# Lillthorin/YoloLite-Official-Repo

Hardware: AMD Instinct MI355X
Metric: images/sec (higher is better)
Workload: dtype f32

## Files before the change

### yololite-official-repo_amd/_lib.py

```python
from __future__ import annotations

import ctypes as C
import os
import sys
import warnings


def _default_hw_queues():
    if "GPU_MAX_HW_QUEUES" in os.environ or os.environ.get("YOLOLITE_NO_ENV_DEFAULTS"):
        return
    os.environ["GPU_MAX_HW_QUEUES"] = "8"
    t = sys.modules.get("torch")
    try:
        late = t is not None and t.cuda.is_initialized()
    except Exception:
        late = False
    if late:
        warnings.warn("yololite_amd: the HIP runtime was initialised before this package was imported, so "
                      "GPU_MAX_HW_QUEUES=8 cannot be applied; export it in the environment (multi-stream overlap "
                      "of the executor degrades by ~25 % next to RCCL streams otherwise)", RuntimeWarning)


_default_hw_queues()

_HERE = os.path.dirname(os.path.abspath(__file__))
LIB_PATH = os.environ.get("YOLOLITE_HIP_LIB") or os.path.join(_HERE, "libyololite_hip.so")

YL_ABI_VERSION = 5
YL_MAX_LEVELS = 8
YL_OK = 0
ACT = {"none": 0, "relu": 1, "relu6": 2, "silu": 3, "gelu": 4, "relu_lab": 5}
OP_STEM, OP_CONV, OP_DW, OP_STEMBLOCK, OP_SE = 0, 1, 2, 3, 4
OP_POOL, OP_COPY, OP_LN, OP_GRN, OP_NHWC4 = 5, 6, 7, 8, 9
POST_MAIN, POST_FALLBACK, POST_EVAL = 0, 1, 2
CENTER = {"v8": 0, "simple": 1}
WH = {"softplus": 0, "v8": 1, "exp": 2}
NMS_TORCHVISION, NMS_GREEDY = 0, 1

DEV_DW_TILE_OFF, DEV_PWS_OFF, DEV_S2C_OFF, DEV_DWC_ALL, DEV_DWT_OFF = 1, 2, 4, 8, 16
DEV_DWT_NOSPLIT = 1 << 10
DEV_WINO_V1 = 1 << 11
DEV_DWL_OFF = 1 << 14
DEV_DWL_ALL = 1 << 15
DEV_DPW_OFF = 1 << 16
DEV_K3W_OFF = 1 << 17
DEV_POISON = 1 << 18
DEV_CHAIN_OFF = 1 << 19
DEV_WINO_SHAPE_SHIFT = 12

_fp = C.POINTER(C.c_float)
_ip = C.POINTER(C.c_int32)


class yl_layer(C.Structure):
    _fields_ = [(n, C.c_int32) for n in (
        "op", "in_slot", "out_slot", "res_slot", "up_slot", "head_level", "cin", "cout",
        "k", "stride", "pad_t", "pad_l", "act", "in_shift", "dw_k", "dw_stride", "dw_pad_t", "dw_pad_l", "dw_act")] + [
        ("w", _fp), ("b", _fp), ("dw_w", _fp), ("dw_b", _fp),
        ("c2", C.c_int32), ("act2", C.c_int32), ("c3", C.c_int32), ("act3", C.c_int32),
        ("w2", _fp), ("b2", _fp), ("w3", _fp), ("b3", _fp), ("scale_slot", C.c_int32), ("reserved0", C.c_int32),
        ("lab_scale", C.c_float), ("lab_bias", C.c_float), ("eps", C.c_float), ("out_ch_off", C.c_int32)]


class yl_model_desc(C.Structure):
    _fields_ = [("abi_version", C.c_int32), ("img_size", C.c_int32), ("in_channels", C.c_int32),
                ("num_classes", C.c_int32), ("num_masks", C.c_int32), ("proto_slot", C.c_int32),
                ("num_levels", C.c_int32),
                ("level_size", C.c_int32 * YL_MAX_LEVELS), ("level_anchors", C.c_int32 * YL_MAX_LEVELS),
                ("num_slots", C.c_int32), ("slot_h", _ip), ("slot_w", _ip), ("slot_c", _ip),
                ("num_layers", C.c_int32), ("layers", C.POINTER(yl_layer))]


class yl_post_cfg(C.Structure):
    _fields_ = [("mode", C.c_int32), ("conf_thr", C.c_float), ("iou_thr", C.c_float),
                ("per_class_cap", C.c_int32), ("topk", C.c_int32), ("max_out", C.c_int32),
                ("center_mode", C.c_int32), ("wh_mode", C.c_int32), ("backmap_dev", C.c_void_p),
                ("fallback_nms", C.c_int32)]


YL_LOSS_MAX_TOPK = 64
# ... 98 lines not shown
```

### yololite-official-repo_amd/csrc/yl_api.hip

```cpp
#include "yl_internal.h"

#include <dlfcn.h>
#include <limits.h>
#include <math.h>
#include <stdio.h>
#include <stddef.h>
#include <string.h>

#include <algorithm>
#include <memory>
#include <chrono>
#include <string>
#include <vector>

#define YL_DW_LDS_MAX (32 * 1024)

namespace {

struct DevLayer {
  yl_layer d;
  float* wp = nullptr;
  float* bias = nullptr;
  float* dw_w = nullptr;
  float* dw_b = nullptr;
// ... 46 lines not shown
  float* level_buf[YL_MAX_LEVELS] = {nullptr};
  float4* ws_boxes = nullptr;
  float* ws_scores = nullptr;
  int* ws_cls = nullptr;
  int* ws_clsws = nullptr;
  int* ws_kept_list = nullptr;
  int* ws_done = nullptr;
  unsigned long long* ws_gkeys = nullptr;
  int gP = 0;
  float* ws_tmp_dets = nullptr;
  int* ws_tmp_idx = nullptr;
  int post_cap_batch = 0;
  unsigned long long* ws_loss_keys = nullptr;
  float* ws_loss_neg = nullptr;
  float* ws_loss_pi = nullptr;
  int* ws_loss_pos = nullptr;
  int loss_cap_batch = 0;
  int* ws_nms_clsws = nullptr;
  unsigned long long* ws_nms_gkeys = nullptr;
  int nms_gP = 0;
  int opt_graph = 0, opt_tile_m = 0, opt_streams = 2;
  int opt_nms_groups = 0;
  int opt_hybrid = 0;
  int small_lo = 0, small_hi = 0;
  int tiny_lo = 0, tiny_hi = 0;
  int opt_batch_levels = 1;
  int opt_winograd = 1;
  int wino_max_hw = 0;
  int opt_fuse_decode = 1;
  int opt_fuse_head = 1;
  int opt_split_k = 0;
  int opt_dev = 0;
  int chain_launches = 0;
  int opt_bf16 = 0;
  hipStream_t work[4] = {nullptr, nullptr, nullptr, nullptr};
  hipEvent_t ev_fork = nullptr, ev_join[4] = {nullptr, nullptr, nullptr, nullptr};
  int opt_lanes = 0;
  std::vector<unsigned char> lane;
  std::vector<int> readers;
  hipStream_t side[4] = {nullptr, nullptr, nullptr, nullptr};
  hipEvent_t ev_la[4] = {nullptr, nullptr, nullptr, nullptr}, ev_lb[4] = {nullptr, nullptr, nullptr, nullptr};
  struct GraphEntry {
    std::vector<hipGraphExec_t> execs;
    int n = 0;
    std::vector<unsigned char> key;
    unsigned long long stamp = 0;
  };
  std::vector<GraphEntry> graphs;
  unsigned long long graph_clock = 0;
  std::shared_ptr<int> weights_owner;
  std::string err;
};

namespace {

bool g_inited[64] = {false};

yl_status fail(yl_ctx* c, yl_status s, const std::string& msg) {
  if (c) c->err = msg;
  return s;
}

#define HIPCHK(ctx, expr)                                                                        \
  do {                                                                                           \
    hipError_t _e = (expr);                                                                      \
    if (_e != hipSuccess) {                                                                      \
// ... 496 lines not shown
};
#define YL_MODE_LAUNCHERS(S, SD)                                                                             \
  {yl_launch_conv##S, yl_launch_conv_multi##S, yl_launch_stem##SD, yl_launch_dw##SD, yl_launch_stemblock##S, \
   yl_launch_stemdw##S, yl_conv_init##S, yl_convc_init##S, yl_stemblock_init##S}
const ModeLaunchers kLaunch[4] = {YL_MODE_LAUNCHERS(, ), YL_MODE_LAUNCHERS(_bf16, ), YL_MODE_LAUNCHERS(_f16, ),
                                  YL_MODE_LAUNCHERS(_f16s, _f16s)};

yl_status launch_failed(yl_ctx* c, const LaunchStep& s, hipError_t e) {
  static const char* const what[] = {"", "batched ", "head ", "expand-only ", "fused ", "chained ", "split head "};
  char b[256];
  snprintf(b, sizeof(b), "layers %zu..%zu %slaunch failed: %s", s.first, s.first + s.layers - 1, what[s.form], hipGetErrorString(e));
  return fail(c, YL_ERR_HIP, b);
}

struct LayerRun {
  yl_ctx* c;
  const float* x; int b0, B; float* const* level_out;
  hipStream_t st; hipEvent_t* evs; int chunk; const yl_post_cfg* fuse; size_t lend;
  bool lanes = false;
  hipStream_t sd = nullptr;
  std::vector<unsigned char> prod;
  bool side_used = false;
  int pooled_slot = -1, pooled_P = 0;

  void decode_targets(size_t i, YlConvP& p) const {
    const int l = c->layers[i].d.head_level, S = c->level_S[l];
    const size_t o = (size_t)b0 * c->N;
    p.dec_boxes = c->ws_boxes + o; p.dec_scores = c->ws_scores + o; p.dec_cls = c->ws_cls + o;
    p.dec_N = c->N; p.dec_off = c->level_off[l] + c->layers[i].head_anchor * S * S; p.dec_C = c->C;
    p.dec_mode = fuse->mode; p.dec_center = fuse->center_mode; p.dec_wh = fuse->wh_mode;
    p.dec_raw = c->NM > 0 ? 1 : 0;
    p.dec_stride = (float)((double)c->img_size / (double)S);
    p.dec_hi = (float)(c->img_size - 1);
  }
  void params(size_t i, YlConvP& p) const {
    layer_params(c, c->layers[i], b0, B, x, level_out, p);
    if (fuse && c->layers[i].d.head_level >= 0) decode_targets(i, p);
  }
};

yl_status run_layer(LayerRun& r, size_t i) {
  yl_ctx* c = r.c;
  const DevLayer& L = c->layers[i];
  const yl_layer& d = L.d;
  const int b0 = r.b0, B = r.B;
  const ModeLaunchers& ml = kLaunch[c->opt_bf16];
  YlConvP p;
  r.params(i, p);
  const int ln = (r.lanes && c->lane[i]) ? 1 : 0;
  hipStream_t ls = ln ? r.sd : r.st;
  if (r.lanes) {
    bool cross = false;
    const int ins[4] = {d.in_slot, d.res_slot, d.up_slot, d.scale_slot};
    for (int k = 0; k < 4; ++k)
      if (ins[k] >= 0 && d.op != YL_OP_STEM && d.op != YL_OP_STEMBLOCK && d.op != YL_OP_NHWC4 && r.prod[ins[k]] != ln) cross = true;
    if (ln == 1 && !r.side_used) cross = true;
    if (cross) {
      hipEvent_t ev = ln ? c->ev_la[r.chunk] : c->ev_lb[r.chunk];
      HIPCHK(c, hipEventRecord(ev, ln ? r.st : r.sd));
      HIPCHK(c, hipStreamWaitEvent(ls, ev, 0));
    }
    if (ln) r.side_used = true;
    if (d.head_level < 0 && d.out_slot >= 0) r.prod[d.out_slot] = (unsigned char)ln;
  }
  hipError_t e;
  switch (d.op) {
// ... 47 lines not shown
      break;
    case YL_OP_STEMBLOCK: e = d.dw_k == 3 ? ml.stemdw(p, ls) : ml.stemblock(p, ls); break;
    default: e = ml.dw(p, ls); break;
  }
  if (e == hipSuccess && YL_ACT_POSTPASS(d.act) && c->opt_bf16 == 3) return fail(c, YL_ERR_UNSUPPORTED, "store_f16: GELU / ReLU + affine passes are fp32-storage only");
  if (e == hipSuccess && YL_ACT_POSTPASS(d.act)) {
    YlOpP q;
    memset(&q, 0, sizeof(q));
    q.x = p.out; q.out = p.out;
    q.B = B; q.OH = L.out_h; q.OW = L.out_w; q.C = d.cout;
    q.act = d.act; q.lab_s = d.lab_scale; q.lab_b = d.lab_bias;
    if (d.res_slot >= 0) q.res = slot_addr(c, d.res_slot, b0);
    e = yl_launch_op(YL_OP_ACTPASS, q, ls);
  }
  if (e != hipSuccess) return launch_failed(c, {F_LAYER, i, 1, 1}, e);
  if (r.evs) HIPCHK(c, hipEventRecord(r.evs[i + 1], r.st));
  return YL_OK;
}

yl_status emit(LayerRun& r, const LaunchStep& s, bool* refused) {
  yl_ctx* c = r.c;
  const size_t i = s.first, n = (size_t)s.width;
  hipError_t e = hipSuccess;
  YlConvP ps[4];
  switch (s.form) {
    case F_LAYER: return run_layer(r, i);
    case F_HEAD_RUN:
      for (size_t q = 0; q < n; ++q) {
        const DevLayer& O = c->layers[i + n + q];
        r.params(i + q, ps[q]);
        ps[q].w3p = O.wp; ps[q].b3 = O.bias; ps[q].C3 = O.d.cout;
        r.decode_targets(i + n + q, ps[q]);
      }
      e = yl_launch_conv_dpp(ps, (int)n, r.st);
      break;
    case F_DPQ_EXPAND:
      r.params(i, ps[0]);
      ps[0].w3p = nullptr;
      e = yl_launch_conv_dpq(ps[0], r.st);
      break;
    case F_DPQ_PAIR: case F_DWX_CHAIN: {
      YlConvP& pt = ps[0]; YlConvP& po = ps[1];
      r.params(i, pt);
      r.params(i + 1, po);
      pt.w3p = po.wp; pt.b3 = po.bias; pt.C3 = po.N; pt.act3 = po.act;
      if (s.form == F_DPQ_PAIR) { pt.res = po.res; pt.out = po.out; }
      e = s.form == F_DPQ_PAIR ? yl_launch_conv_dpq(pt, r.st) : yl_launch_conv_dwx(pt, po.out, r.st);
      if (s.form == F_DWX_CHAIN && e == hipSuccess) ++c->chain_launches;
      break;
    }
    case F_SPLIT_HEAD: case F_BATCHED:
      for (size_t q = 0; q < n; ++q) {
        r.params(i + q, ps[q]);
        if (s.form == F_BATCHED) continue;
        const DevLayer& L = c->layers[i + q];
        YlConvP& a = ps[q];
        const int nd = 5 + c->C;
        a.wp = L.wp_det; a.bias = L.b_det; a.N = nd; a.NTtot = cdiv(nd, 16); a.dec_raw = 0;
        a.w3p = L.wp_mc; a.b3 = L.b_mc; a.C3 = c->NM;
        a.out += nd; a.ldo = c->E;
      }
      e = kLaunch[c->opt_bf16].conv_multi(ps, (int)n, c->opt_tile_m, r.st);
      break;
  }
  const unsigned fused = form_bit(F_HEAD_RUN) | form_bit(F_DPQ_EXPAND) | form_bit(F_DPQ_PAIR) | form_bit(F_DWX_CHAIN);
  *refused = e == hipErrorNotSupported && (fused & form_bit(s.form));
  if (e != hipSuccess && !*refused) return launch_failed(c, s, e);
// ... 353 lines not shown
  return walk_plan(c, j, st, n, segs, nseg, [&](int g, int i, int, int, hipStream_t ws) -> yl_status {
    HIPCHK(c, hipGraphLaunch(ge->execs[first[g] + i], ws));
    return YL_OK;
  });
}

}

extern "C" {

int32_t yl_abi_version(void) { return YL_ABI_VERSION; }

const char* yl_strerror(yl_status s) {
  switch (s) {
    case YL_OK: return "ok";
    case YL_ERR_INVALID: return "invalid argument";
    case YL_ERR_HIP: return "HIP runtime error";
    case YL_ERR_NOMEM: return "out of memory";
    case YL_ERR_STATE: return "invalid state for this call";
    case YL_ERR_UNSUPPORTED: return "unsupported configuration";
    case YL_ERR_CAPACITY: return "output buffer too small";
    default: return "unknown yl_status";
  }
}

const char* yl_last_error(const yl_ctx* ctx) { return ctx ? ctx->err.c_str() : "null context"; }

void yl_destroy(yl_ctx* c) {
  if (!c) return;
  hipSetDevice(c->device);
  free_act(c);
  free_post_ws(c);
  hipFree(c->ws_nms_clsws);
  hipFree(c->ws_loss_keys); hipFree(c->ws_loss_neg); hipFree(c->ws_loss_pi); hipFree(c->ws_loss_pos);
  for (int i = 0; i < 4; ++i) {
    if (c->work[i]) hipStreamDestroy(c->work[i]);
    if (c->ev_join[i]) hipEventDestroy(c->ev_join[i]);
    if (c->side[i]) hipStreamDestroy(c->side[i]);
    if (c->ev_la[i]) hipEventDestroy(c->ev_la[i]);
    if (c->ev_lb[i]) hipEventDestroy(c->ev_lb[i]);
  }
  if (c->ev_fork) hipEventDestroy(c->ev_fork);
  for (int i = 0; i < 3; ++i) if (c->ev_t[i]) hipEventDestroy(c->ev_t[i]);
  hipFree(c->ws_nms_gkeys);
  if (c->weights_owner.use_count() <= 1) {
    hipFree(c->zeros);
    for (auto& L : c->layers) {
      hipFree(L.wp); hipFree(L.bias); hipFree(L.dw_w); hipFree(L.dw_b);
      hipFree(L.w2p); hipFree(L.b2); hipFree(L.w3p); hipFree(L.b3); hipFree(L.wino);
      hipFree(L.wp_det); hipFree(L.b_det); hipFree(L.wp_mc); hipFree(L.b_mc);
    }
  }
  delete c;
}

yl_status yl_clone(const yl_ctx* src, yl_ctx** out) {
  if (!src || !out) return YL_ERR_INVALID;
  *out = nullptr;
  if (hipSetDevice(src->device) != hipSuccess) return YL_ERR_HIP;
  yl_ctx* c = new (std::nothrow) yl_ctx();
  if (!c) return YL_ERR_NOMEM;
  *out = c;
  c->device = src->device;
  c->img_size = src->img_size; c->in_ch = src->in_ch; c->C = src->C; c->L = src->L; c->N = src->N; c->E = src->E;
  c->NM = src->NM; c->proto_slot = src->proto_slot;
  memcpy(c->level_S, src->level_S, sizeof(c->level_S));
// ... 356 lines not shown
  return YL_OK;
}

yl_status yl_set_option(yl_ctx* c, const char* name, int32_t value) {
  if (!c || !name) return YL_ERR_INVALID;
  if (!strcmp(name, "graph")) { c->opt_graph = value ? 1 : 0; drop_graph(c); return YL_OK; }
  if (!strcmp(name, "mfma_bf16")) { if (c->opt_bf16 == 3) free_act(c); c->opt_bf16 = value ? 1 : (c->opt_bf16 == 1 ? 0 : c->opt_bf16); drop_graph(c); return YL_OK; }
  if (!strcmp(name, "mfma_f16")) { if (c->opt_bf16 == 3) free_act(c); c->opt_bf16 = value ? 2 : (c->opt_bf16 == 2 ? 0 : c->opt_bf16); drop_graph(c); return YL_OK; }
  if (!strcmp(name, "store_f16")) {
    const int nv = value ? 3 : (c->opt_bf16 == 3 ? 0 : c->opt_bf16);
    if ((nv == 3) != (c->opt_bf16 == 3)) free_act(c);
    c->opt_bf16 = nv; drop_graph(c); return YL_OK;
  }
  if (!strcmp(name, "nms_groups")) { c->opt_nms_groups = value < 0 ? 0 : (value > YL_NMS_GROUPS ? YL_NMS_GROUPS : value); drop_graph(c); return YL_OK; }
  if (!strcmp(name, "time_split")) {
    c->opt_time_split = value ? 1 : 0;
    for (int i = 0; i < 3 && value; ++i)
      if (!c->ev_t[i]) HIPCHK(c, hipEventCreate(&c->ev_t[i]));
    c->timing_valid = false;
    return YL_OK;
  }
  if (!strcmp(name, "pre_norm")) { c->opt_pre_norm = value ? 1 : 0; return YL_OK; }
  if (!strcmp(name, "reuse_slots")) { c->opt_reuse = value ? 1 : 0; drop_graph(c); return YL_OK; }
  if (!strcmp(name, "hybrid")) { c->opt_hybrid = value < 0 ? 0 : (value > 2 ? 2 : value); drop_graph(c); return YL_OK; }
  if (!strcmp(name, "batch_levels")) { c->opt_batch_levels = value ? 1 : 0; drop_graph(c); return YL_OK; }
  if (!strcmp(name, "fuse_decode")) { c->opt_fuse_decode = value ? 1 : 0; drop_graph(c); return YL_OK; }
  if (!strcmp(name, "fuse_head")) { c->opt_fuse_head = value ? 1 : 0; drop_graph(c); return YL_OK; }
  if (!strcmp(name, "winograd")) { c->opt_winograd = value < 0 ? 0 : (value > 2 ? 2 : value); drop_graph(c); return YL_OK; }
  if (!strcmp(name, "lanes")) { c->opt_lanes = value ? 1 : 0; drop_graph(c); return YL_OK; }
  if (!strcmp(name, "tile_m")) { c->opt_tile_m = value; drop_graph(c); return YL_OK; }
  if (!strcmp(name, "streams")) { c->opt_streams = value < 1 ? 1 : (value > 4 ? 4 : value); drop_graph(c); return YL_OK; }
  if (!strcmp(name, "split_k")) { c->opt_split_k = value ? 1 : 0; drop_graph(c); return YL_OK; }
  if (!strcmp(name, "dev_select")) { c->opt_dev = value & (int)YL_DEV_MASK; drop_graph(c); return YL_OK; }
  return fail(c, YL_ERR_INVALID, std::string("unknown option ") + name);
}

yl_status yl_get_option(const yl_ctx* c, const char* name, int32_t* value) {
  if (!c || !name || !value) return YL_ERR_INVALID;
  const struct { const char* n; int v; } tab[] = {
      {"graph", c->opt_graph}, {"mfma_bf16", c->opt_bf16 == 1}, {"mfma_f16", c->opt_bf16 == 2}, {"store_f16", c->opt_bf16 == 3}, {"nms_groups", c->opt_nms_groups}, {"time_split", c->opt_time_split},
      {"pre_norm", c->opt_pre_norm}, {"reuse_slots", c->opt_reuse}, {"hybrid", c->opt_hybrid}, {"batch_levels", c->opt_batch_levels},
      {"fuse_decode", c->opt_fuse_decode}, {"fuse_head", c->opt_fuse_head}, {"winograd", c->opt_winograd}, {"lanes", c->opt_lanes},
      {"tile_m", c->opt_tile_m}, {"streams", c->opt_streams}, {"dev_select", c->opt_dev}, {"split_k", c->opt_split_k},
      {"chain_launches", c->chain_launches}};
  for (const auto& t : tab)
    if (!strcmp(name, t.n)) { *value = t.v; return YL_OK; }
  return YL_ERR_INVALID;
}

int32_t yl_query_fused_block(int32_t c_in, int32_t c_mid, int32_t c_out, int32_t dw_k, int32_t dw_stride, int32_t out_h,
                             int32_t out_w) {
  if (c_in < 1 || c_mid < 1 || c_out < 1 || out_h < 1 || out_w < 1) return 0;
  if (yl_ir_supported(c_in, c_mid, c_out, dw_k, dw_stride, out_h, out_w)) return 1;
  if (dw_stride == 1 && !(out_h & 3) && !(out_w & 3) && yl_uib_supported(c_in, c_mid, c_out, dw_k)) return 2;
  return 0;
}

int32_t yl_query_dw_prologue(int32_t c_in, int32_t c_out, int32_t dw_k, int32_t dw_stride, int32_t out_h, int32_t out_w) {
  if (c_in < 1 || c_out < 1 || dw_k < 1 || dw_stride < 1 || out_h < 1 || out_w < 1) return 0;
  if (yl_dws_supported(c_in, c_out, dw_k, dw_stride, out_h, out_w)) return 2;
  if ((size_t)(dw_k * dw_k + 1) * c_in * sizeof(float) <= YL_DW_LDS_MAX) return 1;
  return 0;
}

static yl_status forward_impl(yl_ctx* c, const float* x, int B, float* const* level_out, hipStream_t st,
                              float* layer_ms, const yl_post_cfg* cfg, float* dets, int* counts, int* keep_idx = nullptr) {
  if (!c) return YL_ERR_INVALID;
  if (c->layers.empty()) return fail(c, YL_ERR_STATE, "context was created without layers");
  if (!x || B < 1) return fail(c, YL_ERR_INVALID, "bad input");
  HIPCHK(c, hipSetDevice(c->device));
  yl_status s = ensure_act(c, B, layer_ms ? 1 : chunks_for(c, B));
  if (s != YL_OK) return s;
  if (cfg && (s = ensure_post(c, B)) != YL_OK) return s;
  if ((s = poison_act(c, st)) != YL_OK) return s;
  Job j;
  j.x = x; j.B = B; j.cfg = cfg; j.dets = dets; j.counts = counts; j.keep_idx = keep_idx;
  for (int l = 0; l < c->L; ++l) j.outs[l] = (level_out && level_out[l]) ? level_out[l] : c->level_buf[l];
  if (layer_ms) {
    std::vector<hipEvent_t> ev(c->layers.size() + 1);
// ... 289 lines not shown
```

### yololite-official-repo_amd/csrc/yl_dpp.hip

```cpp
#include <stdlib.h>
#include "yl_internal.h"
#include "yl_dev.h"
#include "yl_epi.h"

constexpr int DPP_NW = 8;
constexpr int DPW_NW = 8;
constexpr int DPP_WPE = 2;

struct YlDppLds {
  static constexpr int WSL = 192;
  static constexpr __host__ __device__ int nbuf(int KB) { return (KB % 3 == 0) ? 3 : 2; }
  size_t w3, dw, b1, b3, win, bytes;
  constexpr __host__ __device__ YlDppLds(int KB, int NT1, int NT3, bool bias3, int ring_f4)
      : w3((size_t)KB * NT1 * 256), dw(w3 + (size_t)NT1 * NT3 * 256), b1(dw + 10 * KB * 16), b3(b1 + NT1 * 16),
        win(b3 + (bias3 ? NT3 * 16 : 0)), bytes((win + (size_t)ring_f4 * 4) * 4) {}
  static constexpr __host__ __device__ YlDppLds dpp(int KB, int NT1, int NT3) { return YlDppLds(KB, NT1, NT3, true, 0); }
  static constexpr __host__ __device__ YlDppLds dpw(int KB, int NT1, int NT3) { return YlDppLds(KB, NT1, NT3, true, DPW_NW * nbuf(KB) * WSL); }
  static constexpr __host__ __device__ YlDppLds dpq(int KB, int NC1, int NT3) { return YlDppLds(KB, NC1 * 6, NT3, false, 0); }
};

template <int KB , int NT1 , int NT3 >
__global__ __launch_bounds__(DPP_NW * 64, DPP_WPE) void yl_conv_dpp_kernel(YlConvMulti mp) {
  int yl_k = 0;
  if (mp.n > 1 && (int)blockIdx.x >= mp.p[1].blk0) yl_k = 1;
// ... 92 lines not shown
      }
      yl_mma_step<NT1, 1>(wq, xq, acc1);
      xq[0] = xn;
      asm volatile("" ::: "memory");
    };
#pragma unroll
    for (int kb = 0; kb < KB; kb += 2) {
      block(xb, kb);
      if (kb + 1 < KB) block(xa, kb + 1);
    }
    const int next = tile + DPP_NW;
    if (next < r1) { setup(next); fetch(xa, 0); }
    f32x4 acc3[1][NT3];
#pragma unroll
    for (int nt = 0; nt < NT3; ++nt) acc3[0][nt] = (f32x4){0.f, 0.f, 0.f, 0.f};
#pragma unroll
    for (int kb = 0; kb < NT1; ++kb) {
      f32x4 hq[1];
      hq[0] = yl_clamp4(acc1[0][kb] + *reinterpret_cast<const f32x4*>(b1l + kb * 16 + 4 * kq), lo1, hi1);
      f32x4 wq[NT3];
#pragma unroll
      for (int nt = 0; nt < NT3; ++nt) wq[nt] = w3l[(kb * NT3 + nt) * 64 + lane];
      yl_mma_step<NT3, 1>(wq, hq, acc3);
      asm volatile("" ::: "memory");
    }
    const YlPix pxd[1] = {pxc};
#pragma unroll
    for (int nt = 0; nt < NT3; ++nt) acc3[0][nt] += *reinterpret_cast<const f32x4*>(b3l + nt * 16 + 4 * kq);
    yl_epi_decode<NT3, 1, true, true>(p, acc3, pxd, 0, kq, lane);
    tile = next;
  }
}

template <int KB , int NT1 , int NT3 >
__global__ __launch_bounds__(DPW_NW * 64, DPW_NW / 4) void yl_conv_dpw_kernel(YlConvMulti mp) {
  int yl_k = 0;
  if (mp.n > 1 && (int)blockIdx.x >= mp.p[1].blk0) yl_k = 1;
  if (mp.n > 2 && (int)blockIdx.x >= mp.p[2].blk0) yl_k = 2;
  if (mp.n > 3 && (int)blockIdx.x >= mp.p[3].blk0) yl_k = 3;
  const YlConvP& p = mp.p[yl_k];
  const int bx = (int)blockIdx.x - p.blk0, gx = p.nblk;
  constexpr int Cin = KB * 16;
  constexpr int NBUF = YlDppLds::nbuf(KB), WSL = YlDppLds::WSL;
  constexpr int G = NT1 / 2;
  constexpr int TPG = (9 + G - 1) / G;
  static_assert(NT1 % 2 == 0 && KB % NBUF == 0 && NBUF + 1 <= KB, "yl_conv_dpw_kernel shape");
  extern __shared__ __attribute__((aligned(16))) float dpp_lds[];
  const int tid = threadIdx.x, lane = tid & 63;
  const int wave = __builtin_amdgcn_readfirstlane(tid >> 6);
  const int kq = lane >> 4, pl = lane & 15;
  constexpr YlDppLds L = YlDppLds::dpw(KB, NT1, NT3);
  f32x4* w1l = reinterpret_cast<f32x4*>(dpp_lds);
  f32x4* w3l = reinterpret_cast<f32x4*>(dpp_lds + L.w3);
  float* dwl = dpp_lds + L.dw;
  float* b1l = dpp_lds + L.b1;
  float* b3l = dpp_lds + L.b3;
  f32x4* const winl = reinterpret_cast<f32x4*>(dpp_lds + L.win) + wave * (NBUF * WSL);
  {
    const f32x4* g1 = reinterpret_cast<const f32x4*>(p.wp);
    for (int r = wave; r < KB * NT1; r += DPW_NW) yl_glds16(g1 + r * 64 + lane, w1l + r * 64);
    const f32x4* g3 = reinterpret_cast<const f32x4*>(p.w3p);
    for (int r = wave; r < NT1 * NT3; r += DPW_NW) yl_glds16(g3 + r * 64 + lane, w3l + r * 64);
    yl_glds_floats(p.dw_w, dwl, 9 * Cin, tid, DPW_NW * 64);
    if (p.dw_b) yl_glds_floats(p.dw_b, dwl + 9 * Cin, Cin, tid, DPW_NW * 64);
    else for (int i = tid; i < Cin; i += DPW_NW * 64) dwl[9 * Cin + i] = 0.0f;
    yl_glds_floats(p.bias, b1l, NT1 * 16, tid, DPW_NW * 64);
    yl_glds_floats(p.b3, b3l, NT3 * 16, tid, DPW_NW * 64);
// ... 90 lines not shown
          wq[cur ^ 1][0] = w1l[((kb + 1) * NT1 + 0) * 64 + lane];
          wq[cur ^ 1][1] = w1l[((kb + 1) * NT1 + 1) * 64 + lane];
        } else {
          wq[cur ^ 1][0] = w3l[0 * 64 + lane];
          wq[cur ^ 1][1] = w3l[1 * 64 + lane];
        }
#pragma unroll
        for (int t = 0; t < TPG; ++t)
          if (g * TPG + t < 9) {
            tx[t] = tap_at(bufn, g * TPG + t);
            tv[t] = *reinterpret_cast<const f32x4*>(tapw + (g * TPG + t) * Cin + kbn * 16);
          }
        __builtin_amdgcn_sched_barrier(0);
#pragma unroll
        for (int st = 0; st < 4; ++st) {
          acc1[0][2 * g] = __builtin_amdgcn_mfma_f32_16x16x4f32(wq[cur][0][st], xq[0][st], acc1[0][2 * g], 0, 0, 0);
          acc1[0][2 * g + 1] = __builtin_amdgcn_mfma_f32_16x16x4f32(wq[cur][1][st], xq[0][st], acc1[0][2 * g + 1], 0, 0, 0);
        }
        __builtin_amdgcn_sched_barrier(0);
#pragma unroll
        for (int t = 0; t < TPG; ++t)
          if (g * TPG + t < 9) xn = yl_fma4(tx[t], tv[t], xn);
        __builtin_amdgcn_sched_barrier(0);
      }
      xq[0] = yl_clamp4(xn, dlo, dhi);
      if (kb + 1 + NBUF < KB) request(cs, kb + 1 + NBUF, bufn);
      else request(ns, kb + 1 + NBUF - KB, bufn);
      __builtin_amdgcn_sched_barrier(0);
    }
    f32x4 acc3[1][NT3];
#pragma unroll
    for (int nt = 0; nt < NT3; ++nt) acc3[0][nt] = (f32x4){0.f, 0.f, 0.f, 0.f};
    static_assert(NT3 % 2 == 0 && (KB * G + NT1 * (NT3 / 2)) % 2 == 0, "A-fragment register sets alternate per group");
#pragma unroll
    for (int kb = 0; kb < NT1; ++kb) {
      f32x4 hq[1];
      hq[0] = yl_clamp4(acc1[0][kb] + *reinterpret_cast<const f32x4*>(b1l + kb * 16 + 4 * kq), lo1, hi1);
#pragma unroll
      for (int g = 0; g < NT3 / 2; ++g) {
        const int cur = (KB * G + kb * (NT3 / 2) + g) & 1;
        if (g + 1 < NT3 / 2) {
          wq[cur ^ 1][0] = w3l[(kb * NT3 + 2 * g + 2) * 64 + lane];
          wq[cur ^ 1][1] = w3l[(kb * NT3 + 2 * g + 3) * 64 + lane];
        } else if (kb + 1 < NT1) {
          wq[cur ^ 1][0] = w3l[((kb + 1) * NT3 + 0) * 64 + lane];
          wq[cur ^ 1][1] = w3l[((kb + 1) * NT3 + 1) * 64 + lane];
        } else {
          wq[cur ^ 1][0] = w1l[0 * 64 + lane];
          wq[cur ^ 1][1] = w1l[1 * 64 + lane];
        }
        __builtin_amdgcn_sched_barrier(0);
#pragma unroll
        for (int st = 0; st < 4; ++st) {
          acc3[0][2 * g] = __builtin_amdgcn_mfma_f32_16x16x4f32(wq[cur][0][st], hq[0][st], acc3[0][2 * g], 0, 0, 0);
          acc3[0][2 * g + 1] = __builtin_amdgcn_mfma_f32_16x16x4f32(wq[cur][1][st], hq[0][st], acc3[0][2 * g + 1], 0, 0, 0);
        }
        __builtin_amdgcn_sched_barrier(0);
      }
    }
    const YlPix pxd[1] = {pxc};
#pragma unroll
    for (int nt = 0; nt < NT3; ++nt) acc3[0][nt] += *reinterpret_cast<const f32x4*>(b3l + nt * 16 + 4 * kq);
    yl_epi_decode<NT3, 1, true, true>(p, acc3, pxd, 0, kq, lane);
    tile = next;
    cs = ns; pxc = pxn;
  }
  asm volatile("s_waitcnt vmcnt(0)" ::: "memory");
}

template <int KB , int NC1 , int NT3 >
__global__ __launch_bounds__(DPP_NW * 64, DPP_WPE) void yl_conv_dpq_kernel(YlConvP p) {
  constexpr int Cin = KB * 16, NT1 = NC1 * 6;
  const int bx = (int)blockIdx.x, gx = (int)gridDim.x;
  extern __shared__ __attribute__((aligned(16))) float dpp_lds[];
  const int tid = threadIdx.x, lane = tid & 63;
  const int wave = __builtin_amdgcn_readfirstlane(tid >> 6);
  const int kq = lane >> 4, pl = lane & 15;
  constexpr YlDppLds L = YlDppLds::dpq(KB, NC1, NT3);
  f32x4* w1l = reinterpret_cast<f32x4*>(dpp_lds);
  f32x4* w3l = reinterpret_cast<f32x4*>(dpp_lds + L.w3);
  float* dwl = dpp_lds + L.dw;
  float* b1l = dpp_lds + L.b1;
  {
    const f32x4* g1 = reinterpret_cast<const f32x4*>(p.wp);
    for (int r = wave; r < KB * NT1; r += DPP_NW) yl_glds16(g1 + r * 64 + lane, w1l + r * 64);
    if constexpr (NT3 > 0) {
      const f32x4* g3 = reinterpret_cast<const f32x4*>(p.w3p);
      for (int r = wave; r < NT1 * NT3; r += DPP_NW) yl_glds16(g3 + r * 64 + lane, w3l + r * 64);
    }
    yl_glds_floats(p.dw_w, dwl, 9 * Cin, tid, DPP_NW * 64);
    if (p.dw_b) yl_glds_floats(p.dw_b, dwl + 9 * Cin, Cin, tid, DPP_NW * 64);
    else for (int i = tid; i < Cin; i += DPP_NW * 64) dwl[9 * Cin + i] = 0.0f;
    yl_glds_floats(p.bias, b1l, NT1 * 16, tid, DPP_NW * 64);
  }
  __syncthreads();
  const int H = p.H, W = p.W, OW = p.OW, OH = p.OH, N3 = p.C3;
// ... 276 lines not shown
}

static const YlConvKernel s2c_kernel = yl_conv_s2c_kernel<3, 2>;
static constexpr size_t s2c_lds = YlS2cLds(3, 2).bytes;

bool yl_s2c_supported(int cin, int cout, int c3, int oh, int ow) {
  return cin == 16 && cout == 48 && c3 > 16 && c3 <= 32 && (c3 & 3) == 0 && (oh & 1) == 0 && (ow & 7) == 0;
}

hipError_t yl_launch_conv_s2c(const YlConvP& p, hipStream_t st) {
  if ((p.dev & YL_DEV_S2C_OFF) || !p.w3p || p.k != 3 || p.stride != 2 || p.dw_k || p.C1 > 0 || p.res || p.up || p.in_shift || p.dec_boxes ||
      YL_SMOOTH(p.act) || YL_SMOOTH(p.act3) || !yl_s2c_supported(p.Cin, p.N, p.C3, p.OH, p.OW) ||
      p.OH != (p.H + 2 * p.pad_t - 3) / 2 + 1 || p.OW != (p.W + 2 * p.pad_l - 3) / 2 + 1)
    return hipErrorNotSupported;
  const long t = (long)p.B * (p.OH >> 1) * (p.OW >> 3);
  long nb = YL_NUM_CU;
  if (nb > (t + DPP_NW - 1) / DPP_NW) nb = (t + DPP_NW - 1) / DPP_NW;
  if (nb >= 8) nb &= ~7L;
  hipLaunchKernelGGL(s2c_kernel, dim3((unsigned)nb), dim3(DPP_NW * 64), s2c_lds, st, p);
  return hipGetLastError();
}

#define YL_DPP_SHAPES(X) X(6, 6, 6) X(4, 4, 6)

bool yl_dpp_supported(int cin, int cout, int c3, int oh, int ow) {
  if ((cin & 15) || (cout & 15) || (oh & 3) || (ow & 3)) return false;
#define YL_DPP_CHECK(A, B, C) if (cin == A * 16 && cout == B * 16 && (c3 + 15) / 16 == C) return true;
  YL_DPP_SHAPES(YL_DPP_CHECK)
#undef YL_DPP_CHECK
  return false;
}

template <int KB, int NT1, int NT3>
static hipError_t dpp_go(const YlConvP* ps, int n, hipStream_t st) {
  constexpr size_t lds = YlDppLds::dpp(KB, NT1, NT3).bytes, ldsw = YlDppLds::dpw(KB, NT1, NT3).bytes;
  bool win = !(ps[0].dev & YL_DEV_DPW_OFF);
  for (int k = 0; k < n; ++k) win = win && ps[k].dw_pad_t == 1 && ps[k].dw_pad_l == 1;
  const int nw = win ? DPW_NW : DPP_NW;
  YlConvMulti m;
  m.n = n;
  long total = 0;
  for (int k = 0; k < n; ++k) { m.p[k] = ps[k]; total += (long)ps[k].B * (ps[k].OH >> 2) * (ps[k].OW >> 2); }
  const int budget = YL_NUM_CU;
  int at = 0;
  for (int k = 0; k < n; ++k) {
    const long t = (long)ps[k].B * (ps[k].OH >> 2) * (ps[k].OW >> 2);
    long nb = (t * budget + total / 2) / total;
    if (nb > (t + nw - 1) / nw) nb = (t + nw - 1) / nw;
    nb = (nb + 4) / 8 * 8;
    if (nb < 8) nb = 8;
    m.p[k].blk0 = at;
    m.p[k].nblk = (int)nb;
    at += (int)nb;
  }
  if (win) hipLaunchKernelGGL((yl_conv_dpw_kernel<KB, NT1, NT3>), dim3((unsigned)at), dim3(DPW_NW * 64), ldsw, st, m);
  else hipLaunchKernelGGL((yl_conv_dpp_kernel<KB, NT1, NT3>), dim3((unsigned)at), dim3(DPP_NW * 64), lds, st, m);
  return hipGetLastError();
}

hipError_t yl_launch_conv_dpp(const YlConvP* ps, int n, hipStream_t st) {
  if (n < 1 || n > 4) return hipErrorNotSupported;
  const YlConvP& q = ps[0];
  if (q.k != 1 || q.dw_k != 3 || q.dw_stride != 1 || q.C1 > 0 || q.res || q.up || !q.w3p || !q.dec_boxes || q.dec_raw ||
      YL_SMOOTH(q.act) || YL_SMOOTH(q.dw_act))
    return hipErrorNotSupported;
  for (int k = 0; k < n; ++k)
    if (!yl_dpp_supported(ps[k].Cin, ps[k].N, ps[k].C3, ps[k].OH, ps[k].OW) || ps[k].Cin != q.Cin || ps[k].N != q.N ||
        ps[k].C3 != q.C3 || ps[k].H != ps[k].OH || ps[k].W != ps[k].OW ||
        (size_t)ps[k].B * ps[k].H * ps[k].W * ps[k].Cin * 4 >= ((size_t)1 << 31))
      return hipErrorNotSupported;
  const int kb = q.Cin / 16, nt1 = q.N / 16, nt3 = (q.C3 + 15) / 16;
#define YL_DPP_RUN(A, B, C) if (kb == A && nt1 == B && nt3 == C) return dpp_go<A, B, C>(ps, n, st);
  YL_DPP_SHAPES(YL_DPP_RUN)
#undef YL_DPP_RUN
  return hipErrorNotSupported;
}

#define K3W_NW 8
struct YlK3wLds {
  static constexpr int WSL = YlDppLds::WSL;
  static constexpr __host__ __device__ size_t bytes(int KB) { return (size_t)K3W_NW * KB * WSL * 16; }
};
template <int KB >
__global__ __launch_bounds__(K3W_NW * 64, 2) void yl_conv_k3w_kernel(YlConvP p) {
  constexpr int Cin = KB * 16, WSL = YlK3wLds::WSL;
  extern __shared__ __attribute__((aligned(16))) float dpp_lds[];
  const int tid = threadIdx.x, lane = tid & 63;
  const int wave = __builtin_amdgcn_readfirstlane(tid >> 6);
  const int kq = lane >> 4, pl = lane & 15;
  f32x4* const winl = reinterpret_cast<f32x4*>(dpp_lds) + wave * (KB * WSL);
  f32x4 wr[9][KB];
  {
    const f32x4* const wg = reinterpret_cast<const f32x4*>(p.wp);
#pragma unroll
    for (int tap = 0; tap < 9; ++tap)
#pragma unroll
      for (int kb = 0; kb < KB; ++kb) wr[tap][kb] = wg[(tap * KB + kb) * 64 + lane];
  }
  const int H = p.H, W = p.W, OW = p.OW, OH = p.OH, N = p.N;
  const int tw = OW >> 2, th = OH >> 2;
  const int tiles_img = tw * th;
  const int ntiles = p.B * tiles_img;
  const int bx = blockIdx.x, gx = gridDim.x;
  const YlTileRange tr = yl_band_range(bx, gx, ntiles);
  const int r0 = tr.r0, r1 = tr.r1;
// ... 80 lines not shown

static const YlConvKernel k3w_kernels[2] = {yl_conv_k3w_kernel<1>, yl_conv_k3w_kernel<2>};

static hipError_t k3w_go(const YlConvP& p, hipStream_t st) {
  const int KB = p.Cin / 16;
  const YlConvKernel kern = k3w_kernels[KB - 1];
  const size_t lds = YlK3wLds::bytes(KB);
  const long t = (long)p.B * (p.OH >> 2) * (p.OW >> 2);
  long nb = yl_resident_blocks((const void*)kern, K3W_NW * 64, lds, 2);
  if (nb > (t + K3W_NW - 1) / K3W_NW) nb = (t + K3W_NW - 1) / K3W_NW;
  if (nb >= 8) nb &= ~7L;
  hipLaunchKernelGGL(kern, dim3((unsigned)nb), dim3(K3W_NW * 64), lds, st, p);
  return hipGetLastError();
}

hipError_t yl_launch_conv_k3w(const YlConvP& p, hipStream_t st) {
  if (p.k != 3 || p.stride != 1 || p.pad_t != 1 || p.pad_l != 1 || p.dw_k > 0 || p.C1 > 0 || p.w3p || p.up || p.dec_boxes || p.scale ||
      p.in_shift || p.ldo || (p.N & 3) || p.NTtot != 1 || (p.Cin != 16 && p.Cin != 32) || (p.OH & 3) || (p.OW & 3) || p.H != p.OH || p.W != p.OW ||
      (p.dev & YL_DEV_K3W_OFF))
    return hipErrorNotSupported;
  if (p.wino) return hipErrorNotSupported;
  if ((p.OH >> 2) * (p.OW >> 2) < 1600) return hipErrorNotSupported;
  if ((size_t)p.B * p.H * p.W * p.Cin * 4 >= ((size_t)1 << 31)) return hipErrorNotSupported;
  return k3w_go(p, st);
}

hipError_t yl_dpp_init() {
  hipError_t e = yl_set_lds_cap(s2c_kernel, s2c_lds);
#define YL_DPQ_CAP(A, B, C) if (e == hipSuccess) e = yl_set_lds_cap(yl_conv_dpq_kernel<A, B, C>, YlDppLds::dpq(A, B, C).bytes);
  YL_DPQ_SHAPES(YL_DPQ_CAP)
#undef YL_DPQ_CAP
#define YL_DPP_CAP(A, B, C)                                                                     \
  if (e == hipSuccess) e = yl_set_lds_cap(yl_conv_dpw_kernel<A, B, C>, YlDppLds::dpw(A, B, C).bytes); \
  if (e == hipSuccess) e = yl_set_lds_cap(yl_conv_dpp_kernel<A, B, C>, YlDppLds::dpp(A, B, C).bytes);
  YL_DPP_SHAPES(YL_DPP_CAP)
#undef YL_DPP_CAP
  return e;
}
```

### yololite-official-repo_amd/csrc/yl_internal.h

```cpp
#pragma once
#include <hip/hip_runtime.h>
#include <stdint.h>
#include <map>
#include <mutex>
#include <type_traits>
#include <utility>
#include "../../include/yololite_hip.h"
#include "yl_lp.h"

#define YL_SMOOTH(a) ((a) >= YL_ACT_SILU)
#define YL_ACT_POSTPASS(a) ((a) >= YL_ACT_GELU)

#define YL_NUM_CU 256
#define YL_LDS_KEYS_MAX 16384

struct YlLevels {
  const float* ptr[YL_MAX_LEVELS];
  int S[YL_MAX_LEVELS];
  int A[YL_MAX_LEVELS];
  int off[YL_MAX_LEVELS + 1];
  float stride[YL_MAX_LEVELS];
  int L, N, E, C;
  float hi;
};
// ... 77 lines not shown
  const float* dw_b;
  int B, H, W, Cin;
  int OH, OW, N;
  int k, stride, pad_t, pad_l;
  int act;
  int in_shift;
  int dw_k, dw_stride, dw_pad_t, dw_pad_l, dw_act;
  int MH, MW;
  int KB;
  int TK;
  int NTtot;
  int CH;
  int UH, UW;
  long out_bstride;
  int M;
  int ntiles;
  const float* w2p;
  const float* b2;
  const float* w3p;
  const float* b3;
  int C1, C2, C3, act2, act3;
  int SH, SW;
  int tiles_x, tiles_y;
  int sb_strip;
  float4* dec_boxes;
  float* dec_scores;
  int* dec_cls;
  int dec_N;
  int dec_off;
  int dec_C;
  int dec_mode, dec_center, dec_wh;
  int dec_raw;
  float dec_stride, dec_hi;
  int blk0, nblk;
  const float* wino;
  const float* scale;
  unsigned dev;
  float* pool;
  int pool_wpi;
  int ldo;
  int out_f32;
};

#define YL_DEV_DW_TILE_OFF (1u << 0)
#define YL_DEV_PWS_OFF (1u << 1)
#define YL_DEV_S2C_OFF (1u << 2)
#define YL_DEV_DWC_ALL (1u << 3)
#define YL_DEV_DWT_OFF (1u << 4)
#define YL_DEV_DWK(d) (((d) >> 5) & 3u)
#define YL_DEV_KXK_NW(d) (((d) >> 7) & 3u)
#define YL_DEV_KXK_MT2 (1u << 9)
#define YL_DEV_DWT_NOSPLIT (1u << 10)
#define YL_DEV_WINO_V1 (1u << 11)
#define YL_DEV_WINO_SHAPE(d) (((d) >> 12) & 3u)
#define YL_DEV_DWL_OFF (1u << 14)
#define YL_DEV_DWL_ALL (1u << 15)
#define YL_DEV_DPW_OFF (1u << 16)
#define YL_DEV_K3W_OFF (1u << 17)
#define YL_DEV_POISON (1u << 18)
#define YL_DEV_CHAIN_OFF (1u << 19)
#define YL_DEV_MASK 0x3ffffffu
static_assert(YL_DEV_MASK <= 0x7fffffffu, "dev_select is stored in an int (and an int field of the graph key)");
static_assert(((YL_DEV_DW_TILE_OFF | YL_DEV_PWS_OFF | YL_DEV_S2C_OFF | YL_DEV_DWC_ALL | YL_DEV_DWT_OFF | (3u << 5) | (3u << 7) |
                YL_DEV_KXK_MT2 | YL_DEV_DWT_NOSPLIT | YL_DEV_WINO_V1 | (3u << 12) | YL_DEV_DWL_OFF | YL_DEV_DWL_ALL | YL_DEV_DPW_OFF |
                YL_DEV_K3W_OFF | YL_DEV_POISON | YL_DEV_CHAIN_OFF) & ~YL_DEV_MASK) == 0, "a YL_DEV_* bit lies outside the dev_select mask");

struct YlSeP {
  const float* x;
  float* partial;
  const float* w1;
  const float* b1;
  const float* w2;
  const float* b2;
  float* gate;
  int B, HW, C, RD, P, act;
};
hipError_t yl_launch_se(const YlSeP& p, bool pooled, hipStream_t st);
int yl_se_parts(int HW, int C);
int yl_dw_pool_wpi(int k, int stride, int cin, int n, int oh, int ow);

struct YlOpP {
  const float* x;
  float* out;
  const float* w;
  const float* b;
  float* partial;
  int B, H, W, C, OH, OW;
  int k, stride, pad_t, pad_l;
  int ldo, ch_off;
  int P;
  float eps;
  const float* res;
  int act;
  float lab_s, lab_b;
};
#define YL_OP_ACTPASS 100
hipError_t yl_launch_op(int op, const YlOpP& p, hipStream_t st);
int yl_grn_parts(int HW);
// ... 58 lines not shown

inline int yl_multi_shares(YlConvMulti& m, const long* tiles, int resident, int per_tile_cap) {
  long total = 0;
  for (int k = 0; k < m.n; ++k) total += tiles[k];
  int at = 0;
  for (int k = 0; k < m.n; ++k) {
    long g = ((long)resident * tiles[k] / total + 7) & ~7L;
    const long cap = ((tiles[k] + per_tile_cap - 1) / per_tile_cap + 7) & ~7L;
    if (g > cap) g = cap;
    if (g < 8) g = 8;
    m.p[k].blk0 = at;
    m.p[k].nblk = (int)g;
    at += (int)g;
  }
  if (m.n == 1) m.p[0].nblk = 0;
  return at;
}

#define YL_MODE_PROTOTYPES(S)                                                                                           \
  hipError_t yl_launch_conv##S(const YlConvP& p, int tile_hint, hipStream_t st);                                        \
  hipError_t yl_launch_conv_multi##S(const YlConvP* ps, int n, int tile_hint, hipStream_t st);  \
  hipError_t yl_launch_stem##S(const YlConvP& p, hipStream_t st);                                                       \
  hipError_t yl_launch_dw##S(const YlConvP& p, hipStream_t st);                                                         \
  hipError_t yl_launch_stemblock##S(const YlConvP& p, hipStream_t st);                                                  \
  hipError_t yl_launch_stemdw##S(const YlConvP& p, hipStream_t st);  \
  hipError_t yl_conv_init##S();                                                                                         \
  hipError_t yl_convc_init##S();                                                                                        \
  hipError_t yl_stemblock_init##S();
YL_MODE_PROTOTYPES()
YL_MODE_PROTOTYPES(_bf16)
YL_MODE_PROTOTYPES(_f16)
YL_MODE_PROTOTYPES(_f16s)

hipError_t yl_launch_conv_dpp(const YlConvP* ps, int n, hipStream_t st);
bool yl_dpp_supported(int cin, int cout, int c3, int oh, int ow);
hipError_t yl_dpp_init();
hipError_t yl_launch_conv_s2c(const YlConvP& p, hipStream_t st);
hipError_t yl_launch_conv_dpq(const YlConvP& p, hipStream_t st);
hipError_t yl_launch_conv_k3w(const YlConvP& p, hipStream_t st);
bool yl_dpq_supported(int cin, int cmid, int cout, int oh, int ow);
bool yl_stemblock_supported(int c1, int c2, int c3);
bool yl_uib_supported(int c1, int cmid, int n, int dk);
hipError_t yl_launch_conv_dwc(YlConvMulti& m, hipStream_t st);
hipError_t yl_launch_conv_pwt(const YlConvP& p, hipStream_t st);
hipError_t yl_launch_conv_pwt_multi(const YlConvP* ps, int n, hipStream_t st);
hipError_t yl_launch_conv_ir(const YlConvP& p, hipStream_t st);
bool yl_ir_supported(int c1, int cmid, int n, int dk, int ds, int oh, int ow);
hipError_t yl_launch_conv_pws(const YlConvP& p, hipStream_t st);
hipError_t yl_launch_conv_kxk(const YlConvP& p, hipStream_t st);
hipError_t yl_launch_conv_dwt(YlConvMulti& m, hipStream_t st);
hipError_t yl_launch_conv_dwx(const YlConvP& pd, float* out3, hipStream_t st);
bool yl_dwx_supported(int cin, int cout, int dw_k, int dw_stride, int cout1, int oh, int ow);
hipError_t yl_launch_conv_dwk(const YlConvP& p, hipStream_t st);
hipError_t yl_launch_conv_dws(const YlConvP& p, hipStream_t st);
bool yl_dws_supported(int cin, int n, int dk, int ds, int oh, int ow);
hipError_t yl_launch_conv_wino(const YlConvP& p, hipStream_t st);
```

Before: 48340.

## Skip head box/class GEMM for tiles with no objectness above threshold

In the fused depthwise+pointwise head kernel, the objectness n-tile is computed first. If no pixel in the wavefront passes the confidence threshold, the remaining output GEMM tiles and the decode epilogue are skipped, and those scores are written as -inf. This is meant to cut MFMA work and decode stores for background regions. It adds a wave-wide vote and an optional atomic counter, and leaves the skipped boxes unwritten.

```diff
diff --git a/yololite-official-repo_amd/_lib.py b/yololite-official-repo_amd/_lib.py
--- a/yololite-official-repo_amd/_lib.py
+++ b/yololite-official-repo_amd/_lib.py
@@ -46,6 +46,7 @@
 DEV_K3W_OFF = 1 << 17
 DEV_POISON = 1 << 18
 DEV_CHAIN_OFF = 1 << 19
+DEV_HEAD_SKIP_OFF = 1 << 20
 DEV_WINO_SHAPE_SHIFT = 12
 
 _fp = C.POINTER(C.c_float)
diff --git a/yololite-official-repo_amd/csrc/yl_api.hip b/yololite-official-repo_amd/csrc/yl_api.hip
--- a/yololite-official-repo_amd/csrc/yl_api.hip
+++ b/yololite-official-repo_amd/csrc/yl_api.hip
@@ -102,6 +102,9 @@
   int opt_split_k = 0;
   int opt_dev = 0;
   int chain_launches = 0;
+  int head_skip_launches = 0;
+  int opt_head_skip_count = 0;
+  unsigned* head_skip_cnt = nullptr;
   int opt_bf16 = 0;
   hipStream_t work[4] = {nullptr, nullptr, nullptr, nullptr};
   hipEvent_t ev_fork = nullptr, ev_join[4] = {nullptr, nullptr, nullptr, nullptr};
@@ -664,6 +667,8 @@
     p.dec_raw = c->NM > 0 ? 1 : 0;
     p.dec_stride = (float)((double)c->img_size / (double)S);
     p.dec_hi = (float)(c->img_size - 1);
+    p.dec_conf = fuse->conf_thr;
+    p.dec_skip_cnt = c->opt_head_skip_count ? c->head_skip_cnt : nullptr;
   }
   void params(size_t i, YlConvP& p) const {
     layer_params(c, c->layers[i], b0, B, x, level_out, p);
@@ -777,7 +782,11 @@
         ps[q].w3p = O.wp; ps[q].b3 = O.bias; ps[q].C3 = O.d.cout;
         r.decode_targets(i + n + q, ps[q]);
       }
-      e = yl_launch_conv_dpp(ps, (int)n, r.st);
+      {
+        bool skip_form = false;
+        e = yl_launch_conv_dpp(ps, (int)n, r.st, &skip_form);
+        if (e == hipSuccess && skip_form) ++c->head_skip_launches;
+      }
       break;
     case F_DPQ_EXPAND:
       r.params(i, ps[0]);
@@ -1197,6 +1206,7 @@
   free_act(c);
   free_post_ws(c);
   hipFree(c->ws_nms_clsws);
+  hipFree(c->head_skip_cnt);
   hipFree(c->ws_loss_keys); hipFree(c->ws_loss_neg); hipFree(c->ws_loss_pi); hipFree(c->ws_loss_pos);
   for (int i = 0; i < 4; ++i) {
     if (c->work[i]) hipStreamDestroy(c->work[i]);
@@ -1619,6 +1629,14 @@
   if (!strcmp(name, "streams")) { c->opt_streams = value < 1 ? 1 : (value > 4 ? 4 : value); drop_graph(c); return YL_OK; }
   if (!strcmp(name, "split_k")) { c->opt_split_k = value ? 1 : 0; drop_graph(c); return YL_OK; }
   if (!strcmp(name, "dev_select")) { c->opt_dev = value & (int)YL_DEV_MASK; drop_graph(c); return YL_OK; }
+  if (!strcmp(name, "head_skip_count")) {
+    if (value && !c->head_skip_cnt) {
+      HIPCHK(c, hipSetDevice(c->device));
+      HIPCHK(c, hipMalloc((void**)&c->head_skip_cnt, sizeof(unsigned)));
+      HIPCHK(c, hipMemset(c->head_skip_cnt, 0, sizeof(unsigned)));
+    }
+    c->opt_head_skip_count = value ? 1 : 0; drop_graph(c); return YL_OK;
+  }
   return fail(c, YL_ERR_INVALID, std::string("unknown option ") + name);
 }
 
@@ -1629,9 +1647,19 @@
       {"pre_norm", c->opt_pre_norm}, {"reuse_slots", c->opt_reuse}, {"hybrid", c->opt_hybrid}, {"batch_levels", c->opt_batch_levels},
       {"fuse_decode", c->opt_fuse_decode}, {"fuse_head", c->opt_fuse_head}, {"winograd", c->opt_winograd}, {"lanes", c->opt_lanes},
       {"tile_m", c->opt_tile_m}, {"streams", c->opt_streams}, {"dev_select", c->opt_dev}, {"split_k", c->opt_split_k},
-      {"chain_launches", c->chain_launches}};
+      {"chain_launches", c->chain_launches}, {"head_skip_launches", c->head_skip_launches},
+      {"head_skip_count", c->opt_head_skip_count}};
   for (const auto& t : tab)
     if (!strcmp(name, t.n)) { *value = t.v; return YL_OK; }
+  if (!strcmp(name, "head_skipped_tiles")) {
+    unsigned v = 0;
+    if (c->head_skip_cnt &&
+        (hipSetDevice(c->device) != hipSuccess || hipDeviceSynchronize() != hipSuccess ||
+         hipMemcpy(&v, c->head_skip_cnt, sizeof(v), hipMemcpyDeviceToHost) != hipSuccess))
+      return YL_ERR_HIP;
+    *value = (int32_t)(v & 0x7fffffffu);
+    return YL_OK;
+  }
   return YL_ERR_INVALID;
 }
 
diff --git a/yololite-official-repo_amd/csrc/yl_dpp.hip b/yololite-official-repo_amd/csrc/yl_dpp.hip
--- a/yololite-official-repo_amd/csrc/yl_dpp.hip
+++ b/yololite-official-repo_amd/csrc/yl_dpp.hip
@@ -148,7 +148,7 @@
   }
 }
 
-template <int KB , int NT1 , int NT3 >
+template <int KB , int NT1 , int NT3 , bool SKIP = false>
 __global__ __launch_bounds__(DPW_NW * 64, DPW_NW / 4) void yl_conv_dpw_kernel(YlConvMulti mp) {
   int yl_k = 0;
   if (mp.n > 1 && (int)blockIdx.x >= mp.p[1].blk0) yl_k = 1;
@@ -305,6 +305,71 @@
 #pragma unroll
     for (int nt = 0; nt < NT3; ++nt) acc3[0][nt] = (f32x4){0.f, 0.f, 0.f, 0.f};
     static_assert(NT3 % 2 == 0 && (KB * G + NT1 * (NT3 / 2)) % 2 == 0, "A-fragment register sets alternate per group");
+    const YlPix pxd[1] = {pxc};
+    if constexpr (SKIP) {
+      static_assert(NT3 > 2 && NT1 % 2 == 0, "the skip form needs n-tiles behind the first group, and an even group count in front of them");
+#pragma unroll
+      for (int kb = 0; kb < NT1; ++kb)
+        acc1[0][kb] = yl_clamp4(acc1[0][kb] + *reinterpret_cast<const f32x4*>(b1l + kb * 16 + 4 * kq), lo1, hi1);
+#pragma unroll
+      for (int kb = 0; kb < NT1; ++kb) {
+        const int cur = (KB * G + kb) & 1;
+        if (kb + 1 < NT1) {
+          wq[cur ^ 1][0] = w3l[((kb + 1) * NT3 + 0) * 64 + lane];
+          wq[cur ^ 1][1] = w3l[((kb + 1) * NT3 + 1) * 64 + lane];
+        }
+        __builtin_amdgcn_sched_barrier(0);
+#pragma unroll
+        for (int st = 0; st < 4; ++st) {
+          acc3[0][0] = __builtin_amdgcn_mfma_f32_16x16x4f32(wq[cur][0][st], acc1[0][kb][st], acc3[0][0], 0, 0, 0);
+          acc3[0][1] = __builtin_amdgcn_mfma_f32_16x16x4f32(wq[cur][1][st], acc1[0][kb][st], acc3[0][1], 0, 0, 0);
+        }
+        __builtin_amdgcn_sched_barrier(0);
+      }
+      const float conf = p.dec_conf;
+      const float obj = yl_sigmoid(acc3[0][0].x + b3l[4 * kq]);
+      const bool hit = kq == 1 && pxc.valid && obj > conf;
+      if (conf > 0.0f && !__any(hit)) {
+        wq[0][0] = w1l[0 * 64 + lane];
+        wq[0][1] = w1l[1 * 64 + lane];
+        if (kq == 0 && pxc.valid) {
+          const size_t o = (size_t)pxc.b * p.dec_N + p.dec_off + pxc.oy * p.OW + pxc.ox;
+          p.dec_scores[o] = -INFINITY;
+          p.dec_cls[o] = 0;
+        }
+        if (p.dec_skip_cnt != nullptr && lane == 0) atomicAdd(p.dec_skip_cnt, 1u);
+      } else {
+        wq[0][0] = w3l[2 * 64 + lane];
+        wq[0][1] = w3l[3 * 64 + lane];
+#pragma unroll
+        for (int kb = 0; kb < NT1; ++kb) {
+#pragma unroll
+          for (int g = 1; g < NT3 / 2; ++g) {
+            const int cur = (kb * (NT3 / 2 - 1) + g - 1) & 1;
+            if (g + 1 < NT3 / 2) {
+              wq[cur ^ 1][0] = w3l[(kb * NT3 + 2 * g + 2) * 64 + lane];
+              wq[cur ^ 1][1] = w3l[(kb * NT3 + 2 * g + 3) * 64 + lane];
+            } else if (kb + 1 < NT1) {
+              wq[cur ^ 1][0] = w3l[((kb + 1) * NT3 + 2) * 64 + lane];
+              wq[cur ^ 1][1] = w3l[((kb + 1) * NT3 + 3) * 64 + lane];
+            } else {
+              wq[cur ^ 1][0] = w1l[0 * 64 + lane];
+              wq[cur ^ 1][1] = w1l[1 * 64 + lane];
+            }
+            __builtin_amdgcn_sched_barrier(0);
+#pragma unroll
+            for (int st = 0; st < 4; ++st) {
+              acc3[0][2 * g] = __builtin_amdgcn_mfma_f32_16x16x4f32(wq[cur][0][st], acc1[0][kb][st], acc3[0][2 * g], 0, 0, 0);
+              acc3[0][2 * g + 1] = __builtin_amdgcn_mfma_f32_16x16x4f32(wq[cur][1][st], acc1[0][kb][st], acc3[0][2 * g + 1], 0, 0, 0);
+            }
+            __builtin_amdgcn_sched_barrier(0);
+          }
+        }
+#pragma unroll
+        for (int nt = 0; nt < NT3; ++nt) acc3[0][nt] += *reinterpret_cast<const f32x4*>(b3l + nt * 16 + 4 * kq);
+        yl_epi_decode<NT3, 1, true, true>(p, acc3, pxd, 0, kq, lane);
+      }
+    } else {
 #pragma unroll
     for (int kb = 0; kb < NT1; ++kb) {
       f32x4 hq[1];
@@ -331,10 +396,10 @@
         __builtin_amdgcn_sched_barrier(0);
       }
     }
-    const YlPix pxd[1] = {pxc};
 #pragma unroll
     for (int nt = 0; nt < NT3; ++nt) acc3[0][nt] += *reinterpret_cast<const f32x4*>(b3l + nt * 16 + 4 * kq);
     yl_epi_decode<NT3, 1, true, true>(p, acc3, pxd, 0, kq, lane);
+    }
     tile = next;
     cs = ns; pxc = pxn;
   }
@@ -677,7 +742,7 @@
 }
 
 template <int KB, int NT1, int NT3>
-static hipError_t dpp_go(const YlConvP* ps, int n, hipStream_t st) {
+static hipError_t dpp_go(const YlConvP* ps, int n, hipStream_t st, bool* skip_form) {
   constexpr size_t lds = YlDppLds::dpp(KB, NT1, NT3).bytes, ldsw = YlDppLds::dpw(KB, NT1, NT3).bytes;
   bool win = !(ps[0].dev & YL_DEV_DPW_OFF);
   for (int k = 0; k < n; ++k) win = win && ps[k].dw_pad_t == 1 && ps[k].dw_pad_l == 1;
@@ -698,12 +763,21 @@
     m.p[k].nblk = (int)nb;
     at += (int)nb;
   }
+  const bool skip = win && NT3 > 2 && !(ps[0].dev & YL_DEV_HEAD_SKIP_OFF);
+  if (skip_form) *skip_form = skip;
+  if constexpr (NT3 > 2) {
+    if (skip) {
+      hipLaunchKernelGGL((yl_conv_dpw_kernel<KB, NT1, NT3, true>), dim3((unsigned)at), dim3(DPW_NW * 64), ldsw, st, m);
+      return hipGetLastError();
+    }
+  }
   if (win) hipLaunchKernelGGL((yl_conv_dpw_kernel<KB, NT1, NT3>), dim3((unsigned)at), dim3(DPW_NW * 64), ldsw, st, m);
   else hipLaunchKernelGGL((yl_conv_dpp_kernel<KB, NT1, NT3>), dim3((unsigned)at), dim3(DPP_NW * 64), lds, st, m);
   return hipGetLastError();
 }
 
-hipError_t yl_launch_conv_dpp(const YlConvP* ps, int n, hipStream_t st) {
+hipError_t yl_launch_conv_dpp(const YlConvP* ps, int n, hipStream_t st, bool* skip_form) {
+  if (skip_form) *skip_form = false;
   if (n < 1 || n > 4) return hipErrorNotSupported;
   const YlConvP& q = ps[0];
   if (q.k != 1 || q.dw_k != 3 || q.dw_stride != 1 || q.C1 > 0 || q.res || q.up || !q.w3p || !q.dec_boxes || q.dec_raw ||
@@ -715,7 +789,7 @@
         (size_t)ps[k].B * ps[k].H * ps[k].W * ps[k].Cin * 4 >= ((size_t)1 << 31))
       return hipErrorNotSupported;
   const int kb = q.Cin / 16, nt1 = q.N / 16, nt3 = (q.C3 + 15) / 16;
-#define YL_DPP_RUN(A, B, C) if (kb == A && nt1 == B && nt3 == C) return dpp_go<A, B, C>(ps, n, st);
+#define YL_DPP_RUN(A, B, C) if (kb == A && nt1 == B && nt3 == C) return dpp_go<A, B, C>(ps, n, st, skip_form);
   YL_DPP_SHAPES(YL_DPP_RUN)
 #undef YL_DPP_RUN
   return hipErrorNotSupported;
@@ -862,6 +936,7 @@
 #undef YL_DPQ_CAP
 #define YL_DPP_CAP(A, B, C)                                                                     \
   if (e == hipSuccess) e = yl_set_lds_cap(yl_conv_dpw_kernel<A, B, C>, YlDppLds::dpw(A, B, C).bytes); \
+  if (e == hipSuccess) e = yl_set_lds_cap(yl_conv_dpw_kernel<A, B, C, true>, YlDppLds::dpw(A, B, C).bytes); \
   if (e == hipSuccess) e = yl_set_lds_cap(yl_conv_dpp_kernel<A, B, C>, YlDppLds::dpp(A, B, C).bytes);
   YL_DPP_SHAPES(YL_DPP_CAP)
 #undef YL_DPP_CAP
diff --git a/yololite-official-repo_amd/csrc/yl_internal.h b/yololite-official-repo_amd/csrc/yl_internal.h
--- a/yololite-official-repo_amd/csrc/yl_internal.h
+++ b/yololite-official-repo_amd/csrc/yl_internal.h
@@ -133,6 +133,8 @@
   int dec_mode, dec_center, dec_wh;
   int dec_raw;
   float dec_stride, dec_hi;
+  float dec_conf;
+  unsigned* dec_skip_cnt;
   int blk0, nblk;
   const float* wino;
   const float* scale;
@@ -160,11 +162,12 @@
 #define YL_DEV_K3W_OFF (1u << 17)
 #define YL_DEV_POISON (1u << 18)
 #define YL_DEV_CHAIN_OFF (1u << 19)
+#define YL_DEV_HEAD_SKIP_OFF (1u << 20)
 #define YL_DEV_MASK 0x3ffffffu
 static_assert(YL_DEV_MASK <= 0x7fffffffu, "dev_select is stored in an int (and an int field of the graph key)");
 static_assert(((YL_DEV_DW_TILE_OFF | YL_DEV_PWS_OFF | YL_DEV_S2C_OFF | YL_DEV_DWC_ALL | YL_DEV_DWT_OFF | (3u << 5) | (3u << 7) |
                 YL_DEV_KXK_MT2 | YL_DEV_DWT_NOSPLIT | YL_DEV_WINO_V1 | (3u << 12) | YL_DEV_DWL_OFF | YL_DEV_DWL_ALL | YL_DEV_DPW_OFF |
-                YL_DEV_K3W_OFF | YL_DEV_POISON | YL_DEV_CHAIN_OFF) & ~YL_DEV_MASK) == 0, "a YL_DEV_* bit lies outside the dev_select mask");
+                YL_DEV_K3W_OFF | YL_DEV_POISON | YL_DEV_CHAIN_OFF | YL_DEV_HEAD_SKIP_OFF) & ~YL_DEV_MASK) == 0, "a YL_DEV_* bit lies outside the dev_select mask");
 
 struct YlSeP {
   const float* x;
@@ -289,7 +292,7 @@
 YL_MODE_PROTOTYPES(_f16)
 YL_MODE_PROTOTYPES(_f16s)
 
-hipError_t yl_launch_conv_dpp(const YlConvP* ps, int n, hipStream_t st);
+hipError_t yl_launch_conv_dpp(const YlConvP* ps, int n, hipStream_t st, bool* skip_form = nullptr);
 bool yl_dpp_supported(int cin, int cout, int c3, int oh, int ow);
 hipError_t yl_dpp_init();
 hipError_t yl_launch_conv_s2c(const YlConvP& p, hipStream_t st);
```

Result: faster. 50320, median of 6 (+4.1%).
